# XChenZ/invertAvatar

Measured on AMD Instinct MI355X. Metric: frames/sec (512^2 out, 128^2 neural render); max |dRGB|, higher is better.
Workload: dtype f32 (3x3 convolutions >= 8^2 and the two layers of the ray decoder form their f32 products from fp16 hi/lo pairs on the f16 MFMA -- three products per term, lo x lo ~ 2^-22 dropped -- with f32 accumulation; all other arithmetic f32); 1 GPU; TriPlaneGenerator.synthesis, BASELINE configs[1]: reenact_avatar_next3d single-seed render, 1 frame per synthesis call: 512^2 out, neural_rendering_resolution=128, all three backbones + rasterize + fused renderer + SR 8XDC recomputed every frame; width=full, global_batch=1, parallelism=frame-sharded dp1, collective=none, launch=hipGraph replay (not checked against eager: --full checks it)

## Files before the change

include/ia_hip.h:

```cpp
#ifndef IA_HIP_H_
#define IA_HIP_H_

#include <stddef.h>
#include <stdint.h>

#ifdef __cplusplus
extern "C" {
#endif

#define IA_HIP_ABI_VERSION 7

typedef enum ia_status {
    IA_OK = 0,
    IA_ERR_INVALID_ARG = -1,
    IA_ERR_UNSUPPORTED = -2,
    IA_ERR_LAUNCH = -3,
    IA_ERR_NO_DEVICE = -4
} ia_status;

typedef enum ia_dtype { IA_F32 = 0, IA_F16 = 1, IA_F64 = 2 } ia_dtype;

typedef enum ia_act {
    IA_ACT_LINEAR = 1, IA_ACT_RELU = 2, IA_ACT_LRELU = 3, IA_ACT_TANH = 4, IA_ACT_SIGMOID = 5,
    IA_ACT_ELU = 6, IA_ACT_SELU = 7, IA_ACT_SOFTPLUS = 8, IA_ACT_SWISH = 9
// ... 71 lines not shown
                      float* ray_limits, float* part_scratch, void* stream);
int ia_ray_limits_box_parts(int n_rays);

int ia_importance_stage(const float* z_coarse, const float* w_coarse, float* z_fine, int* inds, int* order,
                        int nrays, void* stream);

int ia_fill_mouth(const float* alpha, float* mouth, int B, int H, int W, void* stream);

int ia_mouth_edge_blur(const float* alpha, const float* mouth, float* out, int B, int H, int W, void* stream);

int ia_rasterize_level(const float* tex_cl, const float* uv, const float* upper_alpha, const float* sta, int64_t sta_batch_stride,
                       float* out, int B, int C, int tex_res, int sta_res, int res, int by0, int by1, int bx0, int bx1, void* stream);

int ia_blend_planes(const float* stitch, const float* full_alpha, const float* static_planes, int64_t sta_batch_stride,
                    float* planes_cl, int B, int y0, int y1, int x0, int x1, void* stream);

int ia_channels_last(const float* x, float* y, int B, int C, int H, int W, void* stream);

int ia_cond_blend(const float* cond, const float* x, float* y, int B, int C, int H, int W, void* stream);

int ia_styles_demod(const float* ws, int B, int num_ws, int w_dim, const int64_t* layer_table, const float* layer_gains,
                    const int* style_row_layer, int style_rows, const int* demod_row_layer, int demod_rows,
                    float* styles, float* demod, void* stream);

int ia_ray_sampler(const float* cam, int cam_stride, float* rays_o, float* rays_d, int B, int resolution, int normalize, void* stream);

int ia_act_split(const float* x, const float* styles, const float* shift, void* xs, int planes, int B, int C, int H, int W, void* stream);

int ia_bn_train_split(const float* x, const float* weight, const float* bias, float* running_mean, float* running_var,
                      long long* num_batches_tracked, double* partials, int chunks, void* xs, int planes, int B, int C, int H, int W,
                      float eps, float momentum, void* stream);

int ia_conv2d_sx_supported(int I, int O, int H, int W, int ksize, int transposed);

int ia_conv2d_mfma_sx(const void* xs, int planes, const void* wk_split, int wk_exp, const float* demod, const float* noise,
                      const float* noise_strength, const float* bias, const float* residual, float* y, void* ys, int ys_planes,
                      const float* styles_next, float* scratch, size_t scratch_bytes, int B, int I, int O, int H, int W,
                      int transposed, int act, float alpha, const float* prelu_alpha, float gain, float clamp, int ksplit, void* stream);

int ia_upsample_bilinear_add(const float* x, const float* addend, float* y, int planes, int H, int W, int OH, int OW, void* stream);

int ia_dwconv3x3_tokens(const float* x, const float* w9c, const float* bias, float* y, int B, int H, int W, int C, int act, void* stream);
int ia_dwconv3x3_tokens_split(const float* x, const float* w9c, const float* bias, void* xs, int B, int H, int W, int C, int act, void* stream);

int ia_conv3x3_s2_tiny_supported(int I, int O, int H, int W);
int ia_conv3x3_s2_tiny(const float* x, const float* w, const float* bias, float* y, int B, int I, int O, int H, int W, int act, float alpha,
                       void* stream);

int ia_conv2d_down_plan(int B, int I, int O, int H, int W, int* h_ksplit, size_t* h_scratch_bytes);
int ia_conv2d_down_sx(const void* xs, int planes, const void* wk_split, int wk_exp, const float* demod, const float* bias, const float* residual,
                      float* y, void* ys, int ys_planes, const float* styles_next, float* scratch, size_t scratch_bytes, int B, int I, int O,
                      int H, int W, int act, float alpha, const float* prelu_alpha, float gain, float clamp, int ksplit, void* stream);

int ia_fir_tail_split(const float* x, const float* f, const float* noise, const float* noise_strength, const float* bias,
                      const float* styles_next, float* y, void* ys, int ys_planes, int n, int c, int in_h, int in_w, int out_h, int out_w,
                      int padx0, int pady0, int flip, float fir_gain, int act, float alpha, float act_gain, float clamp, void* stream);

int ia_conv2d_mfma_sx_rgb(const void* xs, int planes, const void* wk_split, int wk_exp, const float* demod, const float* noise,
                          const float* noise_strength, const float* bias, float* y, void* ys, int ys_planes, const float* styles_next,
                          const float* rgb_wk, const float* rgb_styles, const float* rgb_bias, const float* rgb_residual, float* rgb_out,
                          int rgb_channels, float rgb_clamp, int B, int I, int O, int H, int W, int act, float alpha, float gain, float clamp,
                          void* stream);

int ia_upconv2d_rows_plan(int B, int I, int O, int H, int W, size_t* h_scratch_bytes);
int ia_upconv2d_rows_sx(const void* xs, const void* wk_split, int wk_exp, const float* demod, float* y, float* scratch,
                        size_t scratch_bytes, int B, int I, int O, int H, int W, void* stream);
// ... 260 lines not shown
```

invertavatar_amd/_lib.py:

```python
import ctypes
import os
import threading

import torch

from . import build as _build

_lock = threading.Lock()
_lib = None

c_void_p, c_int, c_int64, c_float = ctypes.c_void_p, ctypes.c_int, ctypes.c_int64, ctypes.c_float
_i64p = ctypes.POINTER(ctypes.c_int64)
_f32p = ctypes.POINTER(ctypes.c_float)

ABI_VERSION = 7

DTYPE_ID = {torch.float32: 0, torch.float16: 1, torch.float64: 2}

_SIGNATURES = {
    'ia_version': [],
    'ia_last_error': [ctypes.c_char_p, ctypes.c_size_t],
    'ia_device_count': [],
    'ia_bias_act': [c_void_p] * 6 + [c_int, c_int64, c_int, c_int64, c_int, c_int, c_float, c_float, c_float, c_void_p],
    'ia_upfirdn2d': [c_void_p, c_void_p, c_void_p, c_int, c_int, c_int, c_int, c_int, _i64p, c_int, c_int, _i64p,
                     c_int, c_int, _i64p] + [c_int] * 7 + [c_float, c_void_p],
    'ia_upfirdn2d_bias_act': [c_void_p] * 6 + [c_int] * 13 + [c_float, c_int, c_float, c_float, c_float, c_void_p],
    'ia_conv2d_mfma': [c_void_p] * 10 + [ctypes.c_size_t] + [c_int] * 8 + [c_float, c_float, c_float, c_int, c_void_p],
    'ia_conv2d_mfma_h': [c_void_p] * 10 + [ctypes.c_size_t] + [c_int] * 8 + [c_float, c_float, c_float, c_int, c_void_p],
    'ia_conv2d_mfma_s': [c_void_p] * 2 + [c_int] + [c_void_p] * 8 + [ctypes.c_size_t] + [c_int] * 8 + [c_float, c_float, c_float, c_int, c_void_p],
    'ia_conv2d_plan': [c_int] * 8 + [ctypes.POINTER(c_int), ctypes.POINTER(ctypes.c_size_t)],
    'ia_modconv_demod': [c_void_p] * 3 + [c_int] * 3 + [c_void_p],
    'ia_render_rays': [c_void_p] * 10 + [c_float, c_float, c_int] + [c_int] * 6 + [c_void_p] * 9 + [c_void_p, c_void_p, c_int] + [c_void_p],
    'ia_render_rays_grid': [c_int, c_int],
    'ia_render_rays_box': [c_void_p] * 6 + [ctypes.c_double, ctypes.c_double] + [c_void_p] * 4 + [c_float, c_float, c_int] + [c_int] * 6 + [c_void_p] * 9 + [c_void_p],
    'ia_ray_limits_box': [c_void_p, c_void_p, ctypes.c_double, c_int, c_int, c_void_p, c_void_p, c_void_p],
    'ia_ray_limits_box_parts': [c_int],
    'ia_importance_stage': [c_void_p] * 5 + [c_int, c_void_p],
    'ia_fill_mouth': [c_void_p, c_void_p, c_int, c_int, c_int, c_void_p],
    'ia_mouth_edge_blur': [c_void_p, c_void_p, c_void_p, c_int, c_int, c_int, c_void_p],
    'ia_conv2d_mfma_sx_rgb': [c_void_p, c_int, c_void_p, c_int] + [c_void_p] * 6 + [c_int] + [c_void_p] * 6 + [c_int, c_float] + [c_int] * 6 + [c_float] * 3 + [c_void_p],
    'ia_conv1x1': [c_void_p] * 6 + [c_int] * 5 + [c_float, c_void_p],
    'ia_torgb_supported': [c_int] * 5,
    'ia_torgb': [c_void_p] * 8 + [c_int] * 5 + [c_float, c_void_p],
    'ia_rasterize_level': [c_void_p] * 4 + [c_int64, c_void_p] + [c_int] * 9 + [c_void_p],
    'ia_blend_planes': [c_void_p] * 3 + [c_int64, c_void_p] + [c_int] * 5 + [c_void_p],
    'ia_channels_last': [c_void_p] * 2 + [c_int] * 4 + [c_void_p],
    'ia_cond_blend': [c_void_p] * 3 + [c_int] * 4 + [c_void_p],
    'ia_split_saturation_poll': [ctypes.POINTER(ctypes.c_uint), c_int, c_void_p],
    'ia_split_saturation_count': [c_void_p, c_int, c_int, c_int, c_int, c_int, c_void_p, c_void_p],
    'ia_act_split': [c_void_p] * 4 + [c_int] * 5 + [c_void_p],
    'ia_conv2d_sx_supported': [c_int] * 6,
    'ia_conv2d_mfma_sx': [c_void_p, c_int, c_void_p, c_int] + [c_void_p] * 7 + [c_int] + [c_void_p] * 2 + [ctypes.c_size_t] + [c_int] * 7 + [c_float, c_void_p, c_float, c_float] + [c_int, c_void_p],
    'ia_bn_train_split': [c_void_p] * 7 + [c_int, c_void_p] + [c_int] * 5 + [c_float, c_float, c_void_p],
    'ia_upsample_bilinear_add': [c_void_p] * 3 + [c_int] * 5 + [c_void_p],
    'ia_dwconv3x3_tokens': [c_void_p] * 4 + [c_int] * 5 + [c_void_p],
    'ia_dwconv3x3_tokens_split': [c_void_p] * 4 + [c_int] * 5 + [c_void_p],
    'ia_conv3x3_s2_tiny_supported': [c_int] * 4,
    'ia_conv3x3_s2_tiny': [c_void_p] * 4 + [c_int] * 6 + [c_float, c_void_p],
    'ia_conv2d_down_plan': [c_int] * 5 + [ctypes.POINTER(c_int), ctypes.POINTER(ctypes.c_size_t)],
    'ia_conv2d_down_sx': [c_void_p, c_int, c_void_p, c_int] + [c_void_p] * 5 + [c_int, c_void_p, c_void_p, ctypes.c_size_t] + [c_int] * 6
                         + [c_float, c_void_p, c_float, c_float, c_int, c_void_p],
    'ia_upconv2d_rows_plan': [c_int] * 5 + [ctypes.POINTER(ctypes.c_size_t)],
    'ia_upconv2d_rows_sx': [c_void_p, c_void_p, c_int, c_void_p, c_void_p, c_void_p, ctypes.c_size_t] + [c_int] * 5 + [c_void_p],
    'ia_upconv2d_fir_sx': [c_void_p, c_int, c_void_p, c_int] + [c_void_p] * 5 + [c_void_p, c_int, c_void_p] + [c_int] * 6 + [c_float] * 3 + [c_void_p],
    'ia_fir_tail_split': [c_void_p] * 8 + [c_int] * 10 + [c_float, c_int, c_float, c_float, c_float, c_void_p],
    'ia_cond_blend_split': [c_void_p] * 4 + [c_int] * 4 + [c_void_p],
    'ia_filtered_lrelu': [c_void_p] * 5 + [c_int] * 17 + [c_float] * 3 + [c_int, c_void_p],
    'ia_convgru_gates': [c_void_p] * 4 + [c_int] * 4 + [c_void_p],
    'ia_convgru_gates_split': [c_void_p] * 4 + [c_int] * 4 + [c_void_p],
    'ia_convgru_update': [c_void_p] * 7 + [c_int] * 4 + [c_void_p],
    'ia_convgru_update_split': [c_void_p] * 7 + [c_int] * 4 + [c_void_p],
    'ia_se_gate': [c_void_p, _i64p, c_void_p, _i64p] + [c_void_p] * 4 + [c_int] * 5 + [c_void_p],
    'ia_se_gate_split': [c_void_p, _i64p, c_void_p, _i64p] + [c_void_p] * 7 + [c_int] * 5 + [c_void_p],
    'ia_attention_supported': [c_int] * 3,
    'ia_attention': [c_void_p] * 4 + [c_int] * 5 + [c_int64] * 8 + [c_float, c_void_p],
    'ia_tokens_split': [c_void_p, c_int64, c_void_p, c_int, c_int, c_void_p],
    'ia_layernorm_split': [c_void_p, c_void_p, c_void_p, c_float, c_void_p, c_int, c_int, c_void_p],
    'ia_tokens_split_t': [c_void_p, c_int64, c_void_p, c_int, c_int, c_int, c_void_p],
    'ia_attention_sx_supported': [c_int] * 3,
    'ia_attention_sx': [c_void_p] * 4 + [c_int] * 4 + [c_float, c_void_p],
    'ia_softmax_split': [c_void_p, c_void_p, c_int, c_int, c_int, c_void_p],
    'ia_matmul_sx': [c_void_p, c_void_p, c_void_p] + [c_int] * 5 + [c_int64, c_int64, c_int, c_int64, c_int64, c_int64, c_int64, c_float, c_void_p],
    'ia_im2col_split': [c_void_p, c_void_p] + [c_int] * 7 + [c_void_p],
    'ia_linear_splitk_plan': [c_int, c_int, c_int, ctypes.POINTER(c_int), ctypes.POINTER(ctypes.c_size_t)],
# ... 164 lines not shown
```

invertavatar_amd/csrc/conv_mfma.hip:

```cpp
#include "conv_common.h"
#include <cstdio>
#include <cstdlib>

namespace {

template <int KS, bool TR, int FO, int FP, int WO, int WP, int CC, int NPOS, bool SK, bool DB, int HM>
__global__ __launch_bounds__(WO * WP * 64, WO * WP == 8 ? 1 : 2) void conv_mfma_kernel(const float* __restrict__ x, const float* __restrict__ wk,
                                                                 const float* __restrict__ styles, float* __restrict__ y,
                                                                 float* __restrict__ slabs, Geo g, Epi e) {
    constexpr int NT = KS * KS;
    constexpr int NPH = TR ? 4 : 1;
    constexpr int BO = 32 * FO * WO, BP = 32 * FP * WP, NTHREADS = WO * WP * 64;
    constexpr int PAD = TR ? 0 : KS / 2;
    constexpr int NACC = NPH * FO * FP * 16;
    extern __shared__ __attribute__((aligned(16))) float lds[];

    const int tid = threadIdx.x, lane = tid & 63, wave = tid >> 6;
    const int l31 = lane & 31, half = lane >> 5;
    const int wo = wave / WP, wp = wave % WP;
    const int b = blockIdx.y, worker = blockIdx.x;
    const int npts = g.GH * g.GW;
    const int64_t U = (int64_t)(g.T - g.T_dp) * g.C;
    const int64_t u_begin = SK ? range_begin(worker, U, g.G) : (int64_t)worker * g.C;
    const int64_t u_end = SK ? range_begin(worker + 1, U, g.G) : u_begin + g.C;
    const int first_tile = (int)(u_begin / g.C);
    const int tile_base = SK ? g.T_dp : 0;

  for (int64_t u = u_begin; u < u_end;) {
    const int tile_l = (int)(u / g.C), c_lo = (int)(u - (int64_t)tile_l * g.C);
    const int c_hi = (int)min((int64_t)g.C, (int64_t)c_lo + (u_end - u));
    u += c_hi - c_lo;
    const int tile = tile_base + tile_l;
    const int o0 = (tile % g.TO) * BO;
// ... 387 lines not shown
    const int npts = transposed ? (H + 1) * (W + 1) : H * W;
    tile_dims(O, H, W, ksize, transposed, form, &p.bo, &p.bp, &p.cc, &p.waves, stride);
    bool force_whole = stride == 2 && p.bo == 32 && O > 32;
    if (form == 3 && !force_whole && !transposed && ksize == 3 && p.waves == 8 && O % 32 == 0) {
        const int64_t t_wide = (int64_t)B * ((npts + 255) / 256) * ((O + 127) / 128), t_narrow = (int64_t)B * ((npts + 255) / 256) * (O / 32);
        constexpr int min_tiles = ia::kNumCU;
        if (t_wide < ia::kNumCU && t_narrow >= min_tiles) { p.bo = 32; p.bp = 256; force_whole = true; }
    }
    p.TO = (O + p.bo - 1) / p.bo;
    p.T = ((npts + p.bp - 1) / p.bp) * p.TO;
    p.C = (I + p.cc - 1) / p.cc;
    const int slots = (p.waves == 8 ? 1 : 2) * ia::kNumCU;
    const int Gb = slots / B > 0 ? slots / B : 1;
    const int rounds = p.T / Gb, R = p.T - rounds * Gb;
    if (force_whole || R == 0 || rounds >= 8 || (rounds >= 1 && 4 * R >= 3 * Gb)) {
        p.T_dp = p.T; p.G = 0;
    } else {
        p.T_dp = rounds * Gb;
        const int64_t Ur = (int64_t)R * p.C;
        const int per = rounds > 0 ? (p.C >= 8 ? p.C / 8 : 1) : 2;
        int64_t G = Ur / per;
        if (G > Gb) G = Gb;
        if (rounds == 0 && npts <= kSmallLayerPoints) {
            constexpr int cap = kSmallLayerWorkers;
            const int64_t lim = p.T > cap ? p.T : cap;
            if (G > lim) G = lim;
        }
        if (G < 1) G = 1;
        p.G = (int)G;
    }
    const int frags = (p.bo / 32) * (p.bp / 32) / p.waves;
    p.slab_floats = (transposed ? 4 : 1) * frags * 16 * p.waves * 64;
    return p;
}

int ia_conv2d_plan_tiles(int B, int I, int O, int H, int W, int ksize, int transposed, int form, int stride, int* bo, int* bp, int* waves, int* T,
                         int* TO, int* C, int* T_dp, int* slab_floats) {
    const Plan p = make_plan(B, I, O, H, W, ksize, transposed, form, stride);
    *bo = p.bo; *bp = p.bp; *waves = p.waves; *T = p.T; *TO = p.TO; *C = p.C; *T_dp = p.T_dp; *slab_floats = p.slab_floats;
    return IA_OK;
}

extern "C" int ia_conv2d_sx_supported(int I, int O, int H, int W, int ksize, int transposed) {
    if (ksize != 3 || I % 8 || O % 8 || H < 1 || W < 1) return 0;
    const int npts = transposed ? (H + 1) * (W + 1) : H * W;
    const int side = 8;
    if ((H < W ? H : W) < side) return 0;
    if (transposed) return npts >= (side + 1) * (side + 1) ? 1 : 0;
    return (O >= 128 && npts >= kSplitMinPoints && W <= 512) ? 1 : 0;
}

static size_t scratch_bytes_for(int B, int G, int slab_floats) { return (size_t)B * G * 2 * slab_floats * sizeof(float); }

extern "C" int ia_conv2d_down_plan(int B, int I, int O, int H, int W, int* h_ksplit, size_t* h_scratch_bytes) {
    IA_REQUIRE(h_ksplit && h_scratch_bytes, "null output pointer");
    IA_REQUIRE(B > 0 && I > 0 && O > 0 && H > 0 && W > 0, "empty tensor");
    const int OH = (H - 1) / 2 + 1, OW = (W - 1) / 2 + 1;
    if (I % 8 || O % 8 || OH * OW < kSplitMinPoints || (OH < OW ? OH : OW) < 8)
        return ia::fail(IA_ERR_UNSUPPORTED, "the stride-2 form takes I %% 8 == 0, O %% 8 == 0 and outputs from 8^2 up (%d -> %d @%dx%d)", I, O, H, W);
    const Plan p = make_plan(B, I, O, OH, OW, 3, 0, 3, 2);
    const bool narrow = p.waves == 8 && p.bp == 256 && p.bo == 32;
    if (p.waves != 8 || (narrow && p.T_dp != p.T))
        return ia::fail(IA_ERR_UNSUPPORTED, "no stride-2 tile for %d -> %d @%dx%d (B %d)", I, O, H, W, B);
    *h_ksplit = p.G;
    *h_scratch_bytes = scratch_bytes_for(B, p.G, p.slab_floats);
    return IA_OK;
// ... 127 lines not shown
```

invertavatar_amd/csrc/conv_split.hip:

```cpp
#include "conv_common.h"
#include "lds_dma.h"
#include "conv_small.h"
#include <cstddef>
#ifndef IA_EPI_RELOAD
#define IA_EPI_RELOAD 1
#endif
#include <cstdlib>

#ifndef IA_ABLATE
#define IA_ABLATE 0
#endif
#ifndef IA_PAIR_TAPS
#define IA_PAIR_TAPS 1
#endif
#ifndef IA_ANTIPHASE
#define IA_ANTIPHASE 1
#endif
#define IA_AB_NODMA (IA_ABLATE == 1 || IA_ABLATE >= 5)
#define IA_AB_NOREAD (IA_ABLATE == 3 || IA_ABLATE >= 5)
#define IA_AB_NOSTORE (IA_ABLATE == 4 || IA_ABLATE >= 5)

namespace {

constexpr size_t kLdsBytes = 160 * 1024;

__global__ __launch_bounds__(256) void act_split_kernel(const float* __restrict__ x, const float* __restrict__ styles, const float* __restrict__ shift,
                                                       h16x8* __restrict__ out, int B, int C, int64_t HW, int planes) {
    const int C8 = C / 8;
    const int64_t total = (int64_t)B * C8 * HW, stride = (int64_t)gridDim.x * blockDim.x;
    ia::SatWatch watch;
    for (int64_t i = (int64_t)blockIdx.x * blockDim.x + threadIdx.x; i < total; i += stride) {
        const int64_t pix = i % HW;
        const int c8 = (int)((i / HW) % C8), b = (int)(i / (HW * C8));
        h16x8 hi, lo;
#pragma unroll
// ... 109 lines not shown
                v[k][0] = t.x; v[k][1] = t.y; v[k][2] = t.z; v[k][3] = t.w;
            } else {
                v[k][0] = xb[k * HW + it];
            }
        }
#pragma unroll
        for (int px = 0; px < PX; ++px) {
            h16x8 hi, lo;
#pragma unroll
            for (int k = 0; k < 8; ++k) {
                const float t = fmaf(v[k][px], a[k], cc[k]);
                if (planes == 2) { _Float16 h, l; ia::split_f16(t, h, l, watch); hi[k] = h; lo[k] = l; }
                else hi[k] = ia::round_f16(t, watch);
            }
            dh[it * PX + px] = hi;
            if (planes == 2) dl[it * PX + px] = lo;
        }
    }
    watch.report();
}

__global__ __launch_bounds__(256) void split_saturation_kernel(const unsigned short* __restrict__ xs, int64_t per_batch_hi, int64_t batch_stride,
                                                              int B, unsigned int* __restrict__ count) {
    unsigned int mine = 0;
    const int64_t total = (int64_t)B * per_batch_hi, stride = (int64_t)gridDim.x * blockDim.x;
    for (int64_t i = (int64_t)blockIdx.x * blockDim.x + threadIdx.x; i < total; i += stride) {
        const int64_t b = i / per_batch_hi, e = i - b * per_batch_hi;
        mine += ((xs[b * batch_stride + e] & 0x7fffu) == 0x7bffu) ? 1u : 0u;
    }
    for (int off = 32; off > 0; off >>= 1) mine += __shfl_xor(mine, off);
    if ((threadIdx.x & 63) == 0 && mine) atomicAdd(count, mine);
}

template <int FO, int FP, int WO, int WP>
__device__ __forceinline__ void store_tile_dual(const f32x16 (&acc)[1][FO][FP], float* __restrict__ y, const Geo& g, const Epi& e,
                                                int b, int o0, int p0, int tid, float* lds_f) {
    constexpr int BO = 32 * FO * WO, NTHREADS = WO * WP * 64;
    const int lane = tid & 63, wave = tid >> 6, l31 = lane & 31, half = lane >> 5;
    const int wo = wave / WP, wp = wave % WP;
    const int npts = g.GH * g.GW;
    const int64_t ohw = (int64_t)g.OH * g.OW;
    const float ns = e.noise ? (e.noise_strength ? *e.noise_strength : 1.f) : 0.f;
    const int OR = e.d2s ? g.O / 4 : g.O;
    const int NB = OR / 32;
    float* c_dm = lds_f;
    float* c_bs = lds_f + BO;
    float* c_sn = lds_f + 2 * BO;
    float* c_sl = lds_f + 3 * BO;
    ia::SatWatch watch;
    const bool lrelu = e.act == IA_ACT_LRELU;
    __syncthreads();
    for (int t = tid; t < BO; t += NTHREADS) {
        const int o = e.d2s ? ((((o0 >> 5) + (t >> 5)) >> 1) % NB) * 32 + (t & 31) : o0 + t;
        const bool ok = o < OR;
        c_dm[t] = (e.demod && ok) ? e.demod[b * OR + o] : 1.f;
        c_bs[t] = (e.bias && ok) ? e.bias[o] : 0.f;
        c_sn[t] = (e.styles_next && ok) ? e.styles_next[b * OR + o] : 1.f;
        c_sl[t] = !lrelu ? 1.f : (e.alpha_vec && ok) ? e.alpha_vec[o] : e.alpha;
    }
    __syncthreads();
    const float clamp = e.clamp >= 0.f ? e.clamp : INFINITY, gain = e.gain;
    const int OW2 = 2 * g.GW;
    const int64_t ohw_out = e.d2s ? 4 * ohw : ohw;
    float* yb = y ? y + ((int64_t)b * OR) * ohw_out : nullptr;
    const float* rb = e.residual ? e.residual + ((int64_t)b * OR) * ohw_out : nullptr;
#pragma unroll
    for (int fp = 0; fp < FP; ++fp) {
        const int p = p0 + (wp * FP + fp) * 32 + l31;
        if (p >= npts) continue;
        const int r = e.d2s ? p / g.GW : 0, c = p - r * g.GW;
#pragma unroll
        for (int fo = 0; fo < FO; ++fo) {
            const int grp = (o0 >> 5) + wo * FO + fo;
            const int64_t pix = e.d2s ? (int64_t)(2 * r + ((grp >> 1) / NB)) * OW2 + 2 * c + (grp & 1) : (int64_t)p;
            const int o_frag = e.d2s ? ((grp >> 1) % NB) * 32 : o0 + (wo * FO + fo) * 32;
            const float nz = e.noise ? e.noise[pix] : 0.f;
#pragma unroll
            for (int q = 0; q < 4; ++q) {
                const int trow = (wo * FO + fo) * 32 + 8 * q + 4 * half, o_first = o_frag + 8 * q + 4 * half;
                const float4 dm4 = *reinterpret_cast<const float4*>(c_dm + trow), bs4 = *reinterpret_cast<const float4*>(c_bs + trow);
                const float4 sn4 = *reinterpret_cast<const float4*>(c_sn + trow), sl4 = *reinterpret_cast<const float4*>(c_sl + trow);
                const float dm[4] = {dm4.x, dm4.y, dm4.z, dm4.w}, bs[4] = {bs4.x, bs4.y, bs4.z, bs4.w}, sn[4] = {sn4.x, sn4.y, sn4.z, sn4.w};
                const float sl[4] = {sl4.x, sl4.y, sl4.z, sl4.w};
                const bool inside = o_first + 3 < OR;
                const int64_t at = (int64_t)o_first * ohw_out + pix;
                float res[4] = {0.f, 0.f, 0.f, 0.f};
                if (rb && inside) {
#pragma unroll
                    for (int k = 0; k < 4; ++k) res[k] = rb[at + k * ohw_out];
                }
                float v[4], t[4];
#pragma unroll
                for (int k = 0; k < 4; ++k) {
                    float a = acc[0][fo][fp][4 * q + k] * dm[k];
                    a = fmaf(nz, ns, a);
                    a += bs[k];
                    a = a > 0.f ? a : a * sl[k];
                    a *= gain;
                    { const float c = fminf(fmaxf(a, -clamp), clamp); a = (a != a) ? a : c; }
                    a += res[k];
                    v[k] = inside ? a : 0.f;
                    t[k] = v[k] * sn[k];
                }
                if (yb && inside) {
#pragma unroll
                    for (int k = 0; k < 4; ++k) yb[at + k * ohw_out] = v[k];
                }
                if (e.ys && inside) split_store4(e.ys, nullptr, e.ys_planes, b, OR, ohw_out, o_first, pix, t, watch);
            }
        }
    }
    watch.report();
}

template <int FO, int FP, int WO, int WP>
__device__ __forceinline__ void store_tile_rgb(const f32x16 (&acc)[1][FO][FP], float* __restrict__ y, const Geo& g, const Epi& e,
                                               int b, int o0, int p0, int tid, float* lds_f) {
    constexpr int BO = 32 * FO * WO, NTHREADS = WO * WP * 64;
    const int lane = tid & 63, wave = tid >> 6, l31 = lane & 31, half = lane >> 5;
    const int wo = wave / WP, wp = wave % WP;
    const int npts = g.GH * g.GW;
    const int64_t ohw = (int64_t)g.OH * g.OW;
    const float ns = e.noise ? (e.noise_strength ? *e.noise_strength : 1.f) : 0.f;
    float* yb = y ? y + ((int64_t)b * g.O) * ohw : nullptr;
    float* ws = lds_f;
    float* red = lds_f + kMaxRgb * BO;
    float* c_dm = red + WO * WP * FP * kMaxRgb * 32;
    float* c_bs = c_dm + BO;
    ia::SatWatchNow watch;
    __syncthreads();
    for (int i = tid; i < kMaxRgb * BO; i += NTHREADS) {
        const int c = i / BO, o = o0 + i - c * BO;
        ws[i] = (c < e.rgb_n && o < g.O) ? e.rgb_w[o * e.rgb_n + c] * (e.rgb_styles ? e.rgb_styles[b * g.O + o] : 1.f) : 0.f;
    }
    for (int t = tid; t < BO; t += NTHREADS) {
        const int o = o0 + t;
        c_dm[t] = (e.demod && o < g.O) ? e.demod[b * g.O + o] : 1.f;
// ... 557 lines not shown
    if (quad)
        hipLaunchKernelGGL(bn_split_kernel<4>, grid, dim3(256), 0, s, x, partials, weight, bias, running_mean, running_var, num_batches_tracked,
                           static_cast<h16x8*>(xs), B, C, HW, chunks, eps, momentum, planes);
    else
        hipLaunchKernelGGL(bn_split_kernel<1>, grid, dim3(256), 0, s, x, partials, weight, bias, running_mean, running_var, num_batches_tracked,
                           static_cast<h16x8*>(xs), B, C, HW, chunks, eps, momentum, planes);
    return ia::check_launch("ia_bn_train_split");
}

extern "C" int ia_split_saturation_count(const void* xs, int planes, int B, int C, int H, int W, unsigned int* count, void* stream) {
    IA_REQUIRE(xs && count, "null pointer argument");
    IA_REQUIRE((planes == 1 || planes == 2) && B > 0 && C > 0 && C % 8 == 0 && H > 0 && W > 0, "not a split tensor shape");
    const int64_t per_plane = (int64_t)C * H * W;
    hipStream_t s = (hipStream_t)stream;
    if (hipMemsetAsync(count, 0, sizeof(unsigned int), s) != hipSuccess) return ia::fail(IA_ERR_LAUNCH, "hipMemsetAsync failed");
    hipLaunchKernelGGL(split_saturation_kernel, dim3(ia::streaming_grid((int64_t)B * per_plane, 256)), dim3(256), 0, s,
                       static_cast<const unsigned short*>(xs), per_plane, (int64_t)planes * per_plane, B, count);
    return ia::check_launch("ia_split_saturation_count");
}

int ia_conv2d_plan_tiles(int B, int I, int O, int H, int W, int ksize, int transposed, int form, int stride, int* bo, int* bp, int* waves, int* T,
                         int* TO, int* C, int* T_dp, int* slab_floats);

struct RgbArgs { const float* w; const float* styles; const float* bias; const float* res; float* out; int n; float clamp; };

static int conv_sx_impl(const void* xs, int planes, const void* wk_split, int wk_exp, const float* demod, const float* noise,
                        const float* noise_strength, const float* bias, const float* residual, float* y, void* ys, int ys_planes,
                        const float* styles_next, float* scratch, size_t scratch_bytes, int B, int I, int O, int H, int W,
                        int transposed, int act, float alpha, float gain, float clamp, int ksplit, void* stream, const RgbArgs& rgb,
                        const float* prelu_alpha = nullptr, int d2s = 0, int stride = 1) {
    IA_REQUIRE(xs && wk_split && (y || ys || rgb.out), "xs, wk and at least one output must be device pointers");
    IA_REQUIRE(stride == 1 || (stride == 2 && !transposed && !d2s && !rgb.out && noise == nullptr), "stride 2: the plain 3x3 convolution with padding 1");
    IA_REQUIRE(B > 0 && I > 0 && O > 0 && H > 0 && W > 0, "empty tensor");
    IA_REQUIRE(I % 8 == 0 && O % 8 == 0, "the split form needs I %% 8 == 0 and O %% 8 == 0");
    IA_REQUIRE(wk_exp >= -14 && wk_exp <= 30, "wk_exp is the power of two the weights were scaled by at pack time");
    IA_REQUIRE((planes == 1 && wk_exp == 0) || planes == 2, "planes: 2 = hi / lo pairs (weights from pack_conv_weight_split), 1 = fp16 operands (wk_exp 0)");
    IA_REQUIRE(!ys || ys_planes == 1 || ys_planes == 2, "ys_planes must be 1 or 2");
    IA_REQUIRE(act == IA_ACT_LINEAR || act == IA_ACT_LRELU, "conv epilogue supports linear and lrelu");
    IA_REQUIRE(ksplit >= 0, "worker count must be >= 0");
    IA_REQUIRE(!transposed || (y && !ys && noise == nullptr && bias == nullptr && residual == nullptr && act == IA_ACT_LINEAR),
               "the transposed form writes the fp32 (2H+1)x(2W+1) image only; FIR + bias_act (+ split) follow in ia_fir_tail_split");
    Geo g;
    g.B = B; g.I = I; g.O = O; g.H = H; g.W = W;
    g.GH = transposed ? H + 1 : H; g.GW = transposed ? W + 1 : W;
    g.OH = transposed ? 2 * H + 1 : H; g.OW = transposed ? 2 * W + 1 : W;
    g.stride = stride;
    if (stride == 2) { g.GH = g.OH = (H - 1) / 2 + 1; g.GW = g.OW = (W - 1) / 2 + 1; }
    IA_REQUIRE((int64_t)B * O * g.OH * g.OW <= INT32_MAX && (int64_t)B * I * H * W <= INT32_MAX, "tensor is too large");
    IA_REQUIRE(!d2s || (!transposed && O % 32 == 0 && residual == nullptr && !rgb.out && !prelu_alpha),
               "the depth-to-space store takes a stride-1 layer of 4 x O/4 channels without residual / fused ToRGB");
    int bo, bp, waves, slab_floats;
    const int st_plan = ia_conv2d_plan_tiles(B, I, O, stride == 2 ? g.GH : H, stride == 2 ? g.GW : W, 3, transposed, 3, stride, &bo, &bp, &waves, &g.T, &g.TO,
                                             &g.C, &g.T_dp, &slab_floats);
    if (st_plan != IA_OK) return st_plan;
    const bool wide = waves == 8;
    IA_REQUIRE(wide || (transposed && bo == 64), "the split form covers 3x3 layers on the two-stage tiles (large stride-1 layers, stride-2 transposed)");
    const bool narrow = wide && bp == 256 && (bo == 32 || (bo == 64 && !transposed));
    IA_REQUIRE(!narrow || g.T_dp == g.T, "the narrow tile families run whole tiles only");
    if (rgb.out && narrow) return ia::fail(IA_ERR_UNSUPPORTED, "the fused ToRGB needs the 128-channel tile");
    if (rgb.out && (transposed || g.TO != 1 || g.T_dp != g.T))
        return ia::fail(IA_ERR_UNSUPPORTED, "the fused ToRGB needs a stride-1 layer whose tiles hold every output channel and run in whole rounds "
                        "(O %d, %d channel tiles, %d of %d tiles in whole rounds)", O, g.TO, g.T_dp, g.T);
    g.G = 0;
    const bool small = g.T_dp < g.T && conv_small_shape(B, I, O, H, W, 3, transposed, stride) && !rgb.out && !d2s;
    if (g.T_dp < g.T && !small) {
        IA_REQUIRE(ksplit >= 1, "this layer has stream-K tiles: pass the worker count from ia_conv2d_plan");
        const int64_t Ur = (int64_t)(g.T - g.T_dp) * g.C;
        g.G = (int)(ksplit > Ur ? Ur : ksplit);
        const size_t need = (size_t)B * g.G * 2 * slab_floats * sizeof(float);
        const bool whole_tiles = Ur % g.G == 0 && (Ur / g.G) % g.C == 0;
        IA_REQUIRE(whole_tiles || (scratch && scratch_bytes >= need), "stream-K needs %zu bytes of scratch, got %zu", need, scratch_bytes);
    }
    g.patch_cap = 0;
    g.acc_scale = ldexpf(1.f, -wk_exp);
    Epi e{demod, noise, noise_strength, bias, residual, act, alpha, gain, clamp, ys, styles_next, ys_planes};
    e.alpha_vec = prelu_alpha;
    e.d2s = d2s;
    if (d2s && (bo != 128 || O % 128 != 0 || g.T_dp != g.T))
        return ia::fail(IA_ERR_UNSUPPORTED, "depth-to-space store: needs whole 128-channel tiles (4 x %d channels, %d-channel tiles, %d of %d tiles whole)",
                        O / 4, bo, g.T_dp, g.T);
    if (rgb.out) {
        IA_REQUIRE(rgb.w && rgb.n >= 1 && rgb.n <= kMaxRgb, "the fused ToRGB takes 1 .. %d output channels and its packed weight", kMaxRgb);
        e.rgb_w = rgb.w; e.rgb_styles = rgb.styles; e.rgb_bias = rgb.bias; e.rgb_res = rgb.res; e.rgb_out = rgb.out; e.rgb_n = rgb.n; e.rgb_clamp = rgb.clamp;
// ... 64 lines not shown
```

invertavatar_amd/hipops.py:

```python
import contextlib
import contextvars
import ctypes
import math
import os
import weakref

import torch

from . import _lib

ACT_ID = {'linear': 1, 'lrelu': 3}

PROFILE = None


class _Timed:
    def __init__(self, family, flops, nbytes, desc=''):
        self.args = (family, float(flops), float(nbytes))
        self.desc = desc

    def __enter__(self):
        if PROFILE is not None:
            self.e0 = torch.cuda.Event(enable_timing=True)
            self.e1 = torch.cuda.Event(enable_timing=True)
# ... 21 lines not shown
    o, i, kh, kw = w.shape
    return w.detach().permute(2, 3, 1, 0).reshape(kh * kw, i, o).contiguous()


def pack_conv_weight_h(w):
    o, i, kh, kw = w.shape
    if i % 8:
        raise RuntimeError('fp16 packing needs in_channels % 8 == 0')
    return w.detach().permute(2, 3, 1, 0).reshape(kh * kw, i // 8, 8, o).permute(0, 1, 3, 2).contiguous().to(torch.float16)


def pack_conv_weight_split(w):
    w = w.detach().float()
    top = float(w.abs().max())
    e = 0 if not (top > 0.0 and math.isfinite(top)) else max(-14, min(30, math.floor(math.log2(32768.0 / top))))
    ws = w * (2.0 ** e)
    hi = ws.to(torch.float16)
    lo = (ws - hi.float()).to(torch.float16)
    out = torch.stack([pack_conv_weight_h(hi), pack_conv_weight_h(lo)]).contiguous()
    out.wk_exp = int(e)
    return out


def conv_h_supported(i, o, h, w, ksize, transposed):
    if ksize != 3 or i % 8 or o % 4:
        return False
    if transposed:
        return (h + 1) * (w + 1) > 320
    return o >= 128 and h * w >= 1024 and w <= 512


def conv_sx_supported(i, o, h, w, ksize, transposed):
    return bool(_lib.load().ia_conv2d_sx_supported(int(i), int(o), int(h), int(w), int(ksize), int(bool(transposed))))


def weight_sq_sum(w):
    return w.detach().float().square().sum(dim=[2, 3]).contiguous()


def modconv_demod(styles, wsq):
    b, i = styles.shape
    o = wsq.shape[0]
    d = torch.empty(b, o, device=styles.device, dtype=torch.float32)
    st = _lib.load().ia_modconv_demod(_p(_f32c(styles, 'styles')), _p(_f32c(wsq, 'wsq')), _p(d), b, i, o, _lib.stream_ptr(styles.device))
    _lib.check(st, 'ia_modconv_demod')
    return d


_default_scratch = {}
_scratch_registry = contextvars.ContextVar('ia_scratch_registry', default=None)


@contextlib.contextmanager
def scratch_owner(registry):
    token = _scratch_registry.set(registry)
    try:
        yield registry
    finally:
        _scratch_registry.reset(token)


def _scratch_buffer(device, nbytes):
    reg = _scratch_registry.get()
    if reg is None:
        reg = _default_scratch
    key = (device, torch.cuda.current_stream(device).cuda_stream)
# ... 183 lines not shown
    out = torch.empty(b, planes, c // 8, h, w, 8, device=x.device, dtype=torch.float16)
    with torch.cuda.device(x.device), _Timed('bn_train_split', 3.0 * x.numel(), 4.0 * x.numel() * 2 + 2.0 * out.numel(), f'B{b} C{c} {h}x{w}'):
        st = _lib.load().ia_bn_train_split(_p(x), _p(weight), _p(bias), _p(running_mean), _p(running_var), _p(num_batches_tracked), _p(partials), chunks,
                                           _p(out), int(planes), b, c, h, w, float(eps), float(momentum), _lib.stream_ptr(x.device))
    _lib.check(st, 'ia_bn_train_split')
    for t in (running_mean, running_var, num_batches_tracked):
        if t is not None:
            torch.autograd.graph.increment_version(t)
    return SplitAct(out, c, consumer)


def conv2d_mfma_sx(xs, wk, demod=None, noise=None, noise_strength=None, bias=None, residual=None, transposed=False, act='linear',
                   alpha=0.2, gain=1.0, clamp=None, want_f32=True, split_for=None, styles_next=None, ksplit=None, split_planes=2, prelu=None,
                   want_split=None):
    if not isinstance(xs, SplitAct):
        raise RuntimeError('xs must be a SplitAct (hipops.act_split or a producing layer)')
    if xs.planes == 2 and not (wk.dtype == torch.float16 and wk.dim() == 5 and wk.shape[0] == 2 and hasattr(wk, 'wk_exp')):
        raise RuntimeError('wk must come from pack_conv_weight_split')
    if xs.planes == 1 and not (wk.dtype == torch.float16 and wk.dim() == 4):
        raise RuntimeError('a one-plane input takes the weights of pack_conv_weight_h')
    b, i, h, w = xs.shape
    o = wk.shape[-2]
    if wk.shape[-4] != 9 or wk.shape[-3] * 8 != i:
        raise RuntimeError(f'packed weight {tuple(wk.shape)} does not match 3x3, in-channels {i}')
    if want_split is None:
        want_split = split_for is not None or styles_next is not None
    if prelu is not None and (_f32c(prelu, 'prelu').numel() != o or act != 'lrelu'):
        raise RuntimeError('prelu: [O] per-channel slopes, with act="lrelu"')
    if transposed and (want_split or not want_f32):
        raise RuntimeError('the transposed form only writes the fp32 image')
    for name, t in (('demod', demod), ('noise', noise), ('bias', bias), ('residual', residual), ('styles_next', styles_next)):
        if t is not None:
            _f32c(t, name)
    lib = _lib.load()
    plan_s, plan_bytes = ctypes.c_int(0), ctypes.c_size_t(0)
    _lib.check(lib.ia_conv2d_plan(b, i, o, h, w, 3, int(transposed), 3, ctypes.byref(plan_s), ctypes.byref(plan_bytes)), 'ia_conv2d_plan')
    nbytes = plan_bytes.value
    if ksplit is None:
        ksplit = plan_s.value
    elif plan_s.value > 0 and ksplit != plan_s.value:
        nbytes = nbytes // plan_s.value * max(int(ksplit), 1)
    oh, ow = (2 * h + 1, 2 * w + 1) if transposed else (h, w)
    dev = xs.data.device
    y = torch.empty(b, o, oh, ow, device=dev, dtype=torch.float32) if want_f32 else None
    ys = torch.empty(b, split_planes, o // 8, oh, ow, 8, device=dev, dtype=torch.float16) if want_split else None
    scratch = _scratch_buffer(dev, nbytes) if nbytes else None
    flops = 2.0 * b * h * w * i * o * 9
    traffic = (2.0 * (xs.data.numel() + wk.numel()) + 4.0 * (y.numel() if want_f32 else 0) + 2.0 * (ys.numel() if want_split else 0)
               + 4.0 * (residual.numel() if residual is not None else 0))
    with torch.cuda.device(dev), _Timed('conv2d_mfma_t' if transposed else 'conv2d_mfma_k3', flops, traffic,
                                        f'B{b} I{i} O{o} {h}x{w} G{ksplit} ' + ('f16x3 dma' if xs.planes == 2 else 'f16 dma')):
        st = lib.ia_conv2d_mfma_sx(_p(xs.data), int(xs.planes), _p(wk), int(getattr(wk, 'wk_exp', 0)), _p(demod), _p(noise), _p(noise_strength),
                                   _p(bias), _p(residual), _p(y), _p(ys), int(split_planes), _p(styles_next), _p(scratch), nbytes, b, i, o, h, w, int(transposed), ACT_ID[act],
                                   float(alpha), _p(prelu), float(gain), float(-1 if clamp is None else clamp), int(ksplit), _lib.stream_ptr(dev))
    _lib.check(st, 'ia_conv2d_mfma_sx')
    out_s = SplitAct(ys, o, split_for) if want_split else None
    if want_f32 and want_split:
        return y, out_s
    return y if want_f32 else out_s


def upsample_bilinear_add(x, addend):
    _f32c(x, 'x')
    _f32c(addend, 'addend')
    b, c, h, w = x.shape
    if addend.shape[:2] != x.shape[:2]:
        raise RuntimeError(f'upsample_bilinear_add: {tuple(x.shape)} onto {tuple(addend.shape)}')
# ... 2085 lines not shown
```

Measured before the change: 400.0 frames/s.

## Add intra-block K-split conv kernel for narrow small-tile 3x3 layers

Adds a 3x3 split-precision MFMA convolution kernel that divides the input-channel reduction across four wave pairs inside one block. The partial sums are reduced through LDS before a ragged-safe epilogue. It is routed only for layers whose normal plan is narrow (32x256 tiles, no k-split) and whose tile count fits within the CU count, so these under-occupied layers keep more waves busy. The cost is an LDS reduction, a larger register ring for prefetch, and possible changes to summation order.

```diff
diff --git a/include/ia_hip.h b/include/ia_hip.h
--- a/include/ia_hip.h
+++ b/include/ia_hip.h
@@ -127,6 +127,9 @@
                       float eps, float momentum, void* stream);
 
 int ia_conv2d_sx_supported(int I, int O, int H, int W, int ksize, int transposed);
+
+int ia_conv_ksplit_mode(int mode);
+int ia_conv2d_ksplit_route(int B, int I, int O, int H, int W);
 
 int ia_conv2d_mfma_sx(const void* xs, int planes, const void* wk_split, int wk_exp, const float* demod, const float* noise,
                       const float* noise_strength, const float* bias, const float* residual, float* y, void* ys, int ys_planes,
diff --git a/invertavatar_amd/_lib.py b/invertavatar_amd/_lib.py
--- a/invertavatar_amd/_lib.py
+++ b/invertavatar_amd/_lib.py
@@ -50,6 +50,8 @@
     'ia_split_saturation_count': [c_void_p, c_int, c_int, c_int, c_int, c_int, c_void_p, c_void_p],
     'ia_act_split': [c_void_p] * 4 + [c_int] * 5 + [c_void_p],
     'ia_conv2d_sx_supported': [c_int] * 6,
+    'ia_conv_ksplit_mode': [c_int],
+    'ia_conv2d_ksplit_route': [c_int] * 5,
     'ia_conv2d_mfma_sx': [c_void_p, c_int, c_void_p, c_int] + [c_void_p] * 7 + [c_int] + [c_void_p] * 2 + [ctypes.c_size_t] + [c_int] * 7 + [c_float, c_void_p, c_float, c_float] + [c_int, c_void_p],
     'ia_bn_train_split': [c_void_p] * 7 + [c_int, c_void_p] + [c_int] * 5 + [c_float, c_float, c_void_p],
     'ia_upsample_bilinear_add': [c_void_p] * 3 + [c_int] * 5 + [c_void_p],
diff --git a/invertavatar_amd/csrc/conv_ksplit.h b/invertavatar_amd/csrc/conv_ksplit.h
--- /dev/null
+++ b/invertavatar_amd/csrc/conv_ksplit.h
@@ -0,0 +1,171 @@
+#pragma once
+#include "conv_common.h"
+#include "conv_small.h"
+
+#ifndef IA_KS_ABLATE
+#define IA_KS_ABLATE 0
+#endif
+
+namespace {
+
+constexpr int kKsWaves = 8, kKsQuarters = 4, kKsBO = 64, kKsBP = 128, kKsDepth = 4;
+constexpr int kKsUnroll = kKsDepth * kPairs;
+constexpr size_t kKsLdsBytes = (size_t)kKsWaves * 4 * 4 * 64 * 4 * sizeof(float);
+
+template <int FO, int FP, int WO, int WP, bool RAGGED>
+__device__ __forceinline__ void store_tile_dual(const f32x16 (&acc)[1][FO][FP], float* __restrict__ y, const Geo& g, const Epi& e,
+                                                int b, int o0, int p0, int tid, float* lds_f);
+
+__global__ __launch_bounds__(kKsWaves * 64) void conv_ksplit_kernel(const h16x8* __restrict__ xs, const h16x8* __restrict__ wk,
+                                                                     float* __restrict__ y, Geo g, Epi e) {
+    constexpr int NT = 9, FO = 2, FP = 2;
+    extern __shared__ __attribute__((aligned(16))) float part[];
+    const int tid = threadIdx.x, lane = tid & 63, wave = __builtin_amdgcn_readfirstlane(tid >> 6);
+    const int l31 = lane & 31, half = lane >> 5;
+    const int wp = wave & 1, kq = wave >> 1;
+    const int b = blockIdx.z, o0 = blockIdx.x * kKsBO, p0 = blockIdx.y * kKsBP;
+    const int HW = g.H * g.W, npts = g.GH * g.GW, I8 = g.I / 8;
+    const int plane_bytes = I8 * HW * 16, wplane_bytes = NT * I8 * g.O * 16;
+    constexpr int kOutside = 0x7ffffff0;
+
+    const char* xb = reinterpret_cast<const char*>(xs + (int64_t)b * 2 * I8 * HW);
+    const __amdgpu_buffer_rsrc_t rx0 = small_rsrc(xb, (unsigned)plane_bytes), rx1 = small_rsrc(xb + (int64_t)plane_bytes, (unsigned)plane_bytes);
+    const char* wb = reinterpret_cast<const char*>(wk);
+    const __amdgpu_buffer_rsrc_t rw0 = small_rsrc(wb, (unsigned)wplane_bytes), rw1 = small_rsrc(wb + (int64_t)wplane_bytes, (unsigned)wplane_bytes);
+
+    int a_off[FO][kPairs], b_off[FP][kPairs];
+#pragma unroll
+    for (int s = 0; s < kPairs; ++s) {
+        const int tap = half ? pair_t1(false, s) : pair_t0(false, s);
+        const int ky = tap / 3, kx = tap - 3 * ky;
+#pragma unroll
+        for (int fo = 0; fo < FO; ++fo) {
+            const int o_ld = o0 + fo * 32 + l31;
+            a_off[fo][s] = (tap == kZeroTap || o_ld >= g.O) ? kOutside : ((tap * I8) * g.O + o_ld) * 16;
+        }
+#pragma unroll
+        for (int fp = 0; fp < FP; ++fp) {
+            const int p = p0 + (wp * FP + fp) * 32 + l31;
+            const int r = p / g.GW, c = p - r * g.GW;
+            const int iy = r + ky - 1, ix = c + kx - 1;
+            const bool ok = tap != kZeroTap && p < npts && iy >= 0 && iy < g.H && ix >= 0 && ix < g.W;
+            b_off[fp][s] = ok ? (iy * g.W + ix) * 16 : kOutside;
+        }
+    }
+
+    f32x16 acc[FO][FP];
+#pragma unroll
+    for (int fo = 0; fo < FO; ++fo)
+#pragma unroll
+        for (int fp = 0; fp < FP; ++fp)
+#pragma unroll
+            for (int r = 0; r < 16; ++r) acc[fo][fp][r] = 0.f;
+
+    const int n_oct = kq < I8 ? (I8 - kq + kKsQuarters - 1) / kKsQuarters : 0;
+    h16x8 ra[kKsDepth][2][FO], rb[kKsDepth][2][FP];
+    auto load_step = [&](int slot, int j, int s) {
+        const bool live = j < n_oct && !(IA_KS_ABLATE == 2 && j > 0);
+        const int c8 = live ? kq + kKsQuarters * j : 0;
+        const int wso = c8 * g.O * 16, pso = c8 * HW * 16;
+        const int dead = live ? 0 : kOutside;
+#pragma unroll
+        for (int fo = 0; fo < FO; ++fo) {
+            const int ao = a_off[fo][s] | dead;
+            ra[slot][0][fo] = load16(rw0, ao, wso);
+            ra[slot][1][fo] = load16(rw1, ao, wso);
+        }
+#pragma unroll
+        for (int fp = 0; fp < FP; ++fp) {
+            const int bo = b_off[fp][s] | dead;
+            rb[slot][0][fp] = load16(rx0, bo, pso);
+            rb[slot][1][fp] = load16(rx1, bo, pso);
+        }
+    };
+    if (n_oct > 0) {
+#pragma unroll
+        for (int u = 0; u < kKsDepth; ++u) {
+            load_step(u, 0, u);
+            __builtin_amdgcn_sched_barrier(0);
+        }
+    }
+    static_assert(kKsDepth < kPairs, "the ring's first fill is k-steps 0 .. kKsDepth - 1 of the first octet");
+    for (int j0 = 0; j0 < n_oct; j0 += kKsUnroll / kPairs) {
+#pragma unroll
+        for (int u = 0; u < kKsUnroll; ++u) {
+            const int slot = u % kKsDepth;
+            const h16x8 a_hi[FO] = {ra[slot][0][0], ra[slot][0][1]}, a_lo[FO] = {ra[slot][1][0], ra[slot][1][1]};
+            const h16x8 b_hi[FP] = {rb[slot][0][0], rb[slot][0][1]}, b_lo[FP] = {rb[slot][1][0], rb[slot][1][1]};
+#if IA_KS_ABLATE == 1
+#pragma unroll
+            for (int q = 0; q < FO; ++q) { asm volatile("" ::"v"(a_hi[q])); asm volatile("" ::"v"(a_lo[q])); }
+#pragma unroll
+            for (int q = 0; q < FP; ++q) { asm volatile("" ::"v"(b_hi[q])); asm volatile("" ::"v"(b_lo[q])); }
+#else
+#pragma unroll
+            for (int fo = 0; fo < FO; ++fo)
+#pragma unroll
+                for (int fp = 0; fp < FP; ++fp) acc[fo][fp] = __builtin_amdgcn_mfma_f32_32x32x16_f16(a_lo[fo], b_hi[fp], acc[fo][fp], 0, 0, 0);
+            h16x8 a_sc[FO];
+#pragma unroll
+            for (int fo = 0; fo < FO; ++fo) a_sc[fo] = a_hi[fo] * (_Float16)(1.0f / kLoScale);
+#pragma unroll
+            for (int fo = 0; fo < FO; ++fo)
+#pragma unroll
+                for (int fp = 0; fp < FP; ++fp) acc[fo][fp] = __builtin_amdgcn_mfma_f32_32x32x16_f16(a_sc[fo], b_lo[fp], acc[fo][fp], 0, 0, 0);
+#pragma unroll
+            for (int fo = 0; fo < FO; ++fo)
+#pragma unroll
+                for (int fp = 0; fp < FP; ++fp) acc[fo][fp] = __builtin_amdgcn_mfma_f32_32x32x16_f16(a_hi[fo], b_hi[fp], acc[fo][fp], 0, 0, 0);
+#endif
+            __builtin_amdgcn_sched_barrier(0);
+            load_step(slot, j0 + (u + kKsDepth) / kPairs, (u + kKsDepth) % kPairs);
+            __builtin_amdgcn_sched_barrier(0);
+        }
+    }
+
+    float4* pw = reinterpret_cast<float4*>(part) + (wave * 16) * 64 + lane;
+#pragma unroll
+    for (int fo = 0; fo < FO; ++fo)
+#pragma unroll
+        for (int fp = 0; fp < FP; ++fp)
+#pragma unroll
+            for (int rq = 0; rq < 4; ++rq)
+                pw[((fo * FP + fp) * 4 + rq) * 64] = make_float4(acc[fo][fp][4 * rq], acc[fo][fp][4 * rq + 1], acc[fo][fp][4 * rq + 2], acc[fo][fp][4 * rq + 3]);
+    __syncthreads();
+    const int fo_m = kq >> 1, fp_m = kq & 1;
+    f32x16 fin[1][1][1];
+#pragma unroll
+    for (int rq = 0; rq < 4; ++rq) {
+        const float4* pr = reinterpret_cast<const float4*>(part) + (kq * 4 + rq) * 64 + lane;
+        float4 v = pr[(wp * 16) * 64];
+#if IA_KS_ABLATE != 3
+#pragma unroll
+        for (int q = 1; q < kKsQuarters; ++q) {
+            const float4 u = pr[((q * 2 + wp) * 16) * 64];
+            v.x += u.x; v.y += u.y; v.z += u.z; v.w += u.w;
+        }
+#endif
+        fin[0][0][0][4 * rq] = v.x * g.acc_scale; fin[0][0][0][4 * rq + 1] = v.y * g.acc_scale;
+        fin[0][0][0][4 * rq + 2] = v.z * g.acc_scale; fin[0][0][0][4 * rq + 3] = v.w * g.acc_scale;
+    }
+#if IA_KS_ABLATE == 4
+    float sink = 0.f;
+#pragma unroll
+    for (int r = 0; r < 16; ++r) sink += fin[0][0][0][r];
+    if (sink == 123.456f) y[0] = sink;
+#else
+    const int tid_epi = (fo_m * 4 + wp * 2 + fp_m) * 64 + lane;
+    store_tile_dual<1, 1, 2, 4, true>(fin, y, g, e, b, o0, p0, tid_epi, part);
+#endif
+}
+
+inline int conv_ksplit_launch(const void* xs, const void* wk_split, float* y, const Geo& g, const Epi& e, hipStream_t s) {
+    const int npts = g.GH * g.GW;
+    auto k = conv_ksplit_kernel;
+    if (const int rs = ia::reserve_lds((const void*)k, kKsLdsBytes, "conv_ksplit")) return rs;
+    hipLaunchKernelGGL(k, dim3((g.O + kKsBO - 1) / kKsBO, (npts + kKsBP - 1) / kKsBP, g.B), dim3(kKsWaves * 64), kKsLdsBytes, s,
+                       static_cast<const h16x8*>(xs), static_cast<const h16x8*>(wk_split), y, g, e);
+    return ia::check_launch("ia_conv2d_mfma_sx(k-split)");
+}
+
+}
diff --git a/invertavatar_amd/csrc/conv_mfma.hip b/invertavatar_amd/csrc/conv_mfma.hip
--- a/invertavatar_amd/csrc/conv_mfma.hip
+++ b/invertavatar_amd/csrc/conv_mfma.hip
@@ -1,4 +1,5 @@
 #include "conv_common.h"
+#include <atomic>
 #include <cstdio>
 #include <cstdlib>
 
@@ -452,6 +453,24 @@
     const int frags = (p.bo / 32) * (p.bp / 32) / p.waves;
     p.slab_floats = (transposed ? 4 : 1) * frags * 16 * p.waves * 64;
     return p;
+}
+
+static std::atomic<int> g_ksplit_mode{1};
+
+extern "C" int ia_conv_ksplit_mode(int mode) {
+    if (mode < 0 || mode > 2) return g_ksplit_mode.load();
+    return g_ksplit_mode.exchange(mode);
+}
+
+extern "C" int ia_conv2d_ksplit_route(int B, int I, int O, int H, int W) {
+    const int mode = g_ksplit_mode.load();
+    if (mode == 0 || B < 1 || I < 8 || I % 8 || O < 1 || H < 1 || W < 1) return 0;
+    if (mode == 2) return 1;
+    if (O % 32 || !ia_conv2d_sx_supported(I, O, H, W, 3, 0)) return 0;
+    const Plan p = make_plan(B, I, O, H, W, 3, 0, 3);
+    const bool narrow = p.waves == 8 && p.bo == 32 && p.bp == 256 && p.T_dp == p.T;
+    const int64_t tiles = (int64_t)B * ((H * W + 127) / 128) * ((O + 63) / 64);
+    return narrow && tiles <= ia::kNumCU ? 1 : 0;
 }
 
 int ia_conv2d_plan_tiles(int B, int I, int O, int H, int W, int ksize, int transposed, int form, int stride, int* bo, int* bp, int* waves, int* T,
diff --git a/invertavatar_amd/csrc/conv_split.hip b/invertavatar_amd/csrc/conv_split.hip
--- a/invertavatar_amd/csrc/conv_split.hip
+++ b/invertavatar_amd/csrc/conv_split.hip
@@ -1,6 +1,7 @@
 #include "conv_common.h"
 #include "lds_dma.h"
 #include "conv_small.h"
+#include "conv_ksplit.h"
 #include <cstddef>
 #ifndef IA_EPI_RELOAD
 #define IA_EPI_RELOAD 1
@@ -176,7 +177,7 @@
     if ((threadIdx.x & 63) == 0 && mine) atomicAdd(count, mine);
 }
 
-template <int FO, int FP, int WO, int WP>
+template <int FO, int FP, int WO, int WP, bool RAGGED = false>
 __device__ __forceinline__ void store_tile_dual(const f32x16 (&acc)[1][FO][FP], float* __restrict__ y, const Geo& g, const Epi& e,
                                                 int b, int o0, int p0, int tid, float* lds_f) {
     constexpr int BO = 32 * FO * WO, NTHREADS = WO * WP * 64;
@@ -229,7 +230,13 @@
                 const bool inside = o_first + 3 < OR;
                 const int64_t at = (int64_t)o_first * ohw_out + pix;
                 float res[4] = {0.f, 0.f, 0.f, 0.f};
-                if (rb && inside) {
+                if constexpr (RAGGED) {
+                    if (rb) {
+#pragma unroll
+                        for (int k = 0; k < 4; ++k)
+                            if (o_first + k < OR) res[k] = rb[at + k * ohw_out];
+                    }
+                } else if (rb && inside) {
 #pragma unroll
                     for (int k = 0; k < 4; ++k) res[k] = rb[at + k * ohw_out];
                 }
@@ -243,10 +250,16 @@
                     a *= gain;
                     { const float c = fminf(fmaxf(a, -clamp), clamp); a = (a != a) ? a : c; }
                     a += res[k];
-                    v[k] = inside ? a : 0.f;
+                    v[k] = (RAGGED ? o_first + k < OR : inside) ? a : 0.f;
                     t[k] = v[k] * sn[k];
                 }
-                if (yb && inside) {
+                if constexpr (RAGGED) {
+                    if (yb) {
+#pragma unroll
+                        for (int k = 0; k < 4; ++k)
+                            if (o_first + k < OR) yb[at + k * ohw_out] = v[k];
+                    }
+                } else if (yb && inside) {
 #pragma unroll
                     for (int k = 0; k < 4; ++k) yb[at + k * ohw_out] = v[k];
                 }
@@ -870,7 +883,8 @@
     IA_REQUIRE(xs && wk_split && (y || ys || rgb.out), "xs, wk and at least one output must be device pointers");
     IA_REQUIRE(stride == 1 || (stride == 2 && !transposed && !d2s && !rgb.out && noise == nullptr), "stride 2: the plain 3x3 convolution with padding 1");
     IA_REQUIRE(B > 0 && I > 0 && O > 0 && H > 0 && W > 0, "empty tensor");
-    IA_REQUIRE(I % 8 == 0 && O % 8 == 0, "the split form needs I %% 8 == 0 and O %% 8 == 0");
+    const bool ks_route = planes == 2 && !transposed && stride == 1 && !d2s && !rgb.out && I % 8 == 0 && ia_conv2d_ksplit_route(B, I, O, H, W) != 0;
+    IA_REQUIRE(I % 8 == 0 && (O % 8 == 0 || (ks_route && !ys)), "the split form needs I %% 8 == 0 and O %% 8 == 0");
     IA_REQUIRE(wk_exp >= -14 && wk_exp <= 30, "wk_exp is the power of two the weights were scaled by at pack time");
     IA_REQUIRE((planes == 1 && wk_exp == 0) || planes == 2, "planes: 2 = hi / lo pairs (weights from pack_conv_weight_split), 1 = fp16 operands (wk_exp 0)");
     IA_REQUIRE(!ys || ys_planes == 1 || ys_planes == 2, "ys_planes must be 1 or 2");
@@ -887,6 +901,15 @@
     IA_REQUIRE((int64_t)B * O * g.OH * g.OW <= INT32_MAX && (int64_t)B * I * H * W <= INT32_MAX, "tensor is too large");
     IA_REQUIRE(!d2s || (!transposed && O % 32 == 0 && residual == nullptr && !rgb.out && !prelu_alpha),
                "the depth-to-space store takes a stride-1 layer of 4 x O/4 channels without residual / fused ToRGB");
+    if (ks_route) {
+        IA_REQUIRE((int64_t)18 * I * O <= INT32_MAX && B <= 65535 && (int64_t)H * W <= (int64_t)65535 * kKsBP, "layer is too large for the K-split tile");
+        g.G = 0; g.C = I / 8; g.TO = (O + kKsBO - 1) / kKsBO; g.T = g.T_dp = g.TO * ((H * W + kKsBP - 1) / kKsBP);
+        g.patch_cap = 0;
+        g.acc_scale = ldexpf(1.f, -wk_exp);
+        Epi e{demod, noise, noise_strength, bias, residual, act, alpha, gain, clamp, ys, styles_next, ys_planes};
+        e.alpha_vec = prelu_alpha;
+        return conv_ksplit_launch(xs, wk_split, y, g, e, (hipStream_t)stream);
+    }
     int bo, bp, waves, slab_floats;
     const int st_plan = ia_conv2d_plan_tiles(B, I, O, stride == 2 ? g.GH : H, stride == 2 ? g.GW : W, 3, transposed, 3, stride, &bo, &bp, &waves, &g.T, &g.TO,
                                              &g.C, &g.T_dp, &slab_floats);
diff --git a/invertavatar_amd/hipops.py b/invertavatar_amd/hipops.py
--- a/invertavatar_amd/hipops.py
+++ b/invertavatar_amd/hipops.py
@@ -77,6 +77,20 @@
 
 def conv_sx_supported(i, o, h, w, ksize, transposed):
     return bool(_lib.load().ia_conv2d_sx_supported(int(i), int(o), int(h), int(w), int(ksize), int(bool(transposed))))
+
+
+CONV_KSPLIT = int(os.environ.get('IA_CONV_KSPLIT', 1))
+
+
+def _apply_conv_ksplit(lib):
+    if lib.ia_conv_ksplit_mode(-1) != int(CONV_KSPLIT):
+        lib.ia_conv_ksplit_mode(int(CONV_KSPLIT))
+
+
+def conv_ksplit_route(b, i, o, h, w):
+    lib = _lib.load()
+    _apply_conv_ksplit(lib)
+    return bool(lib.ia_conv2d_ksplit_route(int(b), int(i), int(o), int(h), int(w)))
 
 
 def weight_sq_sum(w):
@@ -326,7 +340,10 @@
     for name, t in (('demod', demod), ('noise', noise), ('bias', bias), ('residual', residual), ('styles_next', styles_next)):
         if t is not None:
             _f32c(t, name)
+    if want_split and o % 8:
+        raise RuntimeError(f'the split output stores channels in groups of 8 (O = {o})')
     lib = _lib.load()
+    _apply_conv_ksplit(lib)
     plan_s, plan_bytes = ctypes.c_int(0), ctypes.c_size_t(0)
     _lib.check(lib.ia_conv2d_plan(b, i, o, h, w, 3, int(transposed), 3, ctypes.byref(plan_s), ctypes.byref(plan_bytes)), 'ia_conv2d_plan')
     nbytes = plan_bytes.value
```

Result: no change. 399.5 frames/s (median of 2 runs) (-0.1%).
